# vani-nag/OWLRayTracing

Hardware: AMD Instinct MI355X
Metric: kNN queries/sec (10M pts, k=10) (higher is better)
Workload: dtype f32; 1 GPU; TrueKNN on 10000000 uniform-random 3-D points (numpy default_rng(0), [0,1)^3), k=10, start radius 0.25*(k/n)^(1/3)=0.0025; BASELINE.json configs[1]; ranks=1, n_points_total=10000000, k=10, kernel=team_kernel, parallelism=1 GPU

## Files before the change

### owlraytracing_amd/csrc/team_args.h

```cpp
#pragma once
#include <stdint.h>

#include <algorithm>
#include <cstdlib>

#include "lbvh.h"
#include "owlknn.h"

#ifndef TKNN_DIAG_BUILD
#define TKNN_DIAG_BUILD 0
#endif

namespace owlmi {

constexpr int kTeamBlock = 64;
inline int grab_for(int64_t count, int blocks, int turns, int cap) {
  if (const char *g = getenv("TKNN_GRAB")) return std::max(1, atoi(g));
  return (int)std::max<int64_t>(1, std::min<int64_t>(cap, count / ((int64_t)std::max(1, blocks) * 4 * turns)));
}
#ifndef TKNN_NREG3
#define TKNN_NREG3 1
#endif
inline int nreg_for(int k) { return k <= 16 ? 1 : (k <= 32 ? 2 : (k <= 48 && TKNN_NREG3 ? 3 : 4)); }

struct TeamArgs {
  LbvhView bvh, halo;
  LbvhWideView wide[2];
  float start_radius;
  const float *start_radii;
  int k;
  int max_rounds;
  int allow_unfinished;
  int first_step;
  int first_ext;
  int merge_ext;
  int count_flat_max;
  int lite;
  float tie_span;
  int diag;
  int32_t ngroups;
  int32_t *out_idx;
  float *out_dist;
  int64_t *out_isect;
  tknnNeigh *out_fb;
  int32_t *out_level;
  uint8_t *done;
  int64_t *isect_sorted;
  int32_t *next_level;
  uint8_t *tie;
  int32_t *tie_list;
  const uint8_t *skip;
  int32_t skip_is;
  const int32_t *slot_count;
  int grab;
  const int32_t *row_slot;
  unsigned long long *counters;
};

}
```

### owlraytracing_amd/csrc/trueknn_team.hip

```cpp
#include "knn_thresholds.h"
#include "team_args.h"
#include "team_lanes.h"
#include "team_walk.h"
#include "trueknn_engine.h"

#include <algorithm>
#include <cmath>
#include <cstdio>
#include <cstdlib>
#include <cstring>
#include <type_traits>

namespace owlmi {

namespace {

#ifndef TKNN_MAX_BLOCKS_3
#define TKNN_MAX_BLOCKS_3 256
#endif
#ifndef TKNN_MAX_BLOCKS_4
#define TKNN_MAX_BLOCKS_4 512
#endif
constexpr int max_blocks(int nreg) { return nreg == 4 ? TKNN_MAX_BLOCKS_4 : (nreg == 3 ? TKNN_MAX_BLOCKS_3 : 256); }
#ifndef TKNN_MAX_PER_QUERY
// ... 17 lines not shown
}
#ifndef TKNN_SORT_FIRST
#define TKNN_SORT_FIRST 1
#endif
#ifndef TKNN_TEAM_WAVES
#define TKNN_TEAM_WAVES 4
#endif
constexpr int kXcdCounter = kDbStats, kXcdCounterStride = 32;
constexpr int kTeamStack = 192;
constexpr int kQrecStride = 6;
constexpr int kScanBudget = 16384;
constexpr int kMaxStep = 2;
constexpr int kCountFlatGroups = 3;
constexpr int kLdsQrec = 64 * kQrecStride * 4;
constexpr int kLdsCnt = 64 * 2 * 4;
constexpr int kLdsList = 64 * 4 + 16;
constexpr int kLdsStack = kTeamStack * 4;
constexpr int kLdsShared = (kLdsCnt + kLdsList) > kLdsStack ? (kLdsCnt + kLdsList) : kLdsStack;
constexpr int kLdsSharedPadded = (kLdsShared + 15) & ~15;
constexpr int kCandCap = kCandCapacity;
template <int NREG>
struct TeamLayout {
  static constexpr int kMaxPerQuery = max_per_query(NREG);
  static constexpr int kMaxBlocks = max_blocks(NREG);
  static constexpr int kLdsBlk = kMaxBlocks * 4;
  static constexpr int kLdsMask = 64 * kMaxPerQuery;
  static constexpr int kHiWords = kMaxBlocks > 256 ? (kMaxPerQuery + 31) / 32 : 0;
  static constexpr int kLdsHi = 64 * kHiWords * 4;
  static constexpr int kEntStride = kMaxPerQuery + 4;
  static constexpr int kLdsEnt = 4 * kEntStride * 4;
  static constexpr int kLdsCand = 4 * kCandCap * 8;
  static constexpr int kOffMask = kLdsQrec + kLdsBlk;
  static constexpr int kOffHi = kOffMask + kLdsMask;
  static constexpr int kOffShared = kOffHi + kLdsHi;
  static constexpr int kOffEnt = kOffShared + kLdsSharedPadded;
  static constexpr int kOffCand = kOffEnt + kLdsEnt;
  static constexpr int kTeamLds = kOffCand + kLdsCand;
  static_assert(kEntStride % 4 == 0 && kOffEnt % 16 == 0, "entry lists must be 16-byte aligned");
  static_assert(kLdsMask % 4 == 0, "the ninth bits are words");
  static_assert(kMaxPerQuery <= 124 && kMaxPerQuery / 4 < 32, "list-length buckets of the pass lists are one bit each of a 32-bit word");
};

struct TeamLds {
  float *qrec;
  int32_t *blk;
  uint8_t *qblk;
  uint32_t *qhi;
  uint32_t *qcnt;
  int32_t *qlist;
  int32_t *ent;
  unsigned long long *cand;
};

template <bool SELECT, bool HALO, int NREG, bool FULL, bool TWO>
__device__ __forceinline__ void team_pass(const TeamArgs &a, const TeamLds &L, int n_list, int32_t first_slot,
                                          const LbvhPoint *own_pts, const LbvhPoint *halo_pts, int lane) {
  const int team = lane >> 4, tl = lane & 15;
  constexpr int kMaxPerQuery = TeamLayout<NREG>::kMaxPerQuery, kEntStride = TeamLayout<NREG>::kEntStride;
  static_assert(!(SELECT && TWO), "only a COUNT pass serves two levels");
  n_list = __builtin_amdgcn_readfirstlane(n_list);
  [[maybe_unused]] unsigned long long tp[4] = {0, 0, 0, 0};
  for (int r0 = 0; r0 < n_list; r0 += 4) {
    [[maybe_unused]] unsigned long long tp_mark = 0;
    if (TKNN_DIAG_BUILD && (a.diag & 128)) tp_mark = __builtin_amdgcn_s_memtime();
#define TP_LAP(i)                                                     \
  do {                                                                \
    if (TKNN_DIAG_BUILD && (a.diag & 128)) {                          \
      const unsigned long long now_ = __builtin_amdgcn_s_memtime();   \
      tp[i] += now_ - tp_mark;                                        \
      tp_mark = now_;                                                 \
    }                                                                 \
  } while (0)
    const bool on = r0 + team < n_list;
    int qi = 0;
    if (on) qi = L.qlist[r0 + team];
    bool lite_q = false;
    if (SELECT && NREG == 1) {
      lite_q = (qi >> 8) != 0;
      qi &= 0xff;
    }
    if (TKNN_DIAG_BUILD && SELECT && (a.diag & 128)) {
      const unsigned long long q_m = __ballot(on && tl == 0), l_m = __ballot(on && tl == 0 && lite_q);
      if (lane == 0) {
        atomicAdd(&a.counters[18], 1ull);
        atomicAdd(&a.counters[19], (unsigned long long)__popcll(q_m));
        atomicAdd(&a.counters[20], (unsigned long long)__popcll(l_m));
      }
    }
    const float *rec = L.qrec + qi * kQrecStride;
    const float t_qx = rec[0], t_qy = rec[1], t_qz = rec[2];
    const int32_t t_qid = __float_as_int(rec[3]);
    const float t_r = rec[4];
    const float t_mg = (fmaxf(fmaxf(fabsf(t_qx), fabsf(t_qy)), fabsf(t_qz)) + 2.0f * t_r) * 4.76837158203125e-07f;
    const float in_below = t_r - t_mg, in_upto = t_r + t_mg;
    const float r_inner = t_r * 0.5f;
    const float i0_below = r_inner - t_mg, i0_upto = r_inner + t_mg;
    uint32_t cnt_i0 = 0;
    const int packed = __float_as_int(rec[5]);
    [[maybe_unused]] int32_t out_row = 0;
    if (SELECT) out_row = a.bvh.prim_id[first_slot + qi];
    const int my_n = on ? (packed & 0xff) : 0;
    const int steps = max(max((int)__builtin_amdgcn_readlane(my_n, 0), (int)__builtin_amdgcn_readlane(my_n, 16)),
                          max((int)__builtin_amdgcn_readlane(my_n, 32), (int)__builtin_amdgcn_readlane(my_n, 48)));
    if (TKNN_DIAG_BUILD && (a.diag & 16) && lane == 0) atomicAdd(&a.counters[15], (unsigned long long)steps);
    const uint8_t *mine = L.qblk + qi * kMaxPerQuery;
    const int last = my_n - 1;
    const int32_t nan_block = a.wide[0].count[0];
    const int own_pos = (packed >> 8) & 0xff;
    const int n_near = (packed >> 16) & 0xff;
    const int last_near = n_near ? n_near - 1 : last;
    const int both = min(own_pos, last_near - own_pos);
    const bool right_longer = last_near - own_pos > own_pos;
    auto list_pos = [&](int it) -> int {
      if (!SELECT) return it;
      const int half = (it + 1) >> 1;
      const int alt = (it & 1) ? half : -half;
      const int far = it - both;
      const int off = it <= 2 * both ? alt : (right_longer ? far : -far);
      return it > last_near ? it : own_pos + off;
    };
    auto list_entry = [&](int pos) -> int32_t {
      int lp = list_pos(pos);
      if (n_near && lp >= n_near) lp = kMaxPerQuery - 1 - (lp - n_near);
      const int at = min(max(lp, 0), kMaxPerQuery - 1);
      int slot_at = mine[at];
      if (TeamLayout<NREG>::kHiWords) slot_at |= (int)((L.qhi[qi * TeamLayout<NREG>::kHiWords + (at >> 5)] >> (at & 31)) & 1u) << 8;
      int32_t e = L.blk[slot_at];
      if (TKNN_DIAG_BUILD && (a.diag & 64)) e = L.blk[mine[0]];
      return resolve_entry<HALO>(pos <= last ? e : nan_block);
    };
    const int steps4 = (steps + 3) & ~3;
    int32_t *my_ent = L.ent + team * kEntStride;
    const bool lite_round = SELECT && NREG == 1 && steps <= a.count_flat_max && __ballot(on && !lite_q) == 0ull;
    if (lite_round) {
      static_assert(4 * kCountFlatGroups + 4 <= 16, "one entry per lane of the team, the group of prefetch included");
      int32_t e = L.blk[mine[tl]];
      if (TKNN_DIAG_BUILD && (a.diag & 64)) e = L.blk[mine[0]];
      my_ent[tl] = resolve_entry<HALO>(tl <= last ? e : nan_block);
    } else {
      for (int base = 0; base < steps4 + 4; base += 16)
        if (base + tl < kEntStride) my_ent[base + tl] = list_entry(base + tl);
    }
    t_wave_sync();
    uint32_t cnt = 0;
    uint32_t bd[NREG], bi[NREG];
#pragma unroll
    for (int j = 0; j < NREG; j++) {
      bd[j] = 0x7f7fffffu;
      bi[j] = 0u;
    }
    constexpr bool full = FULL;
    uint32_t left_out = 0xffffffffu;
    auto kth_dist = [&]() -> float {
      uint32_t reg = bd[0];
#pragma unroll
      for (int j = 1; j < NREG; j++) reg = ((a.k - 1) >> 4) == j ? bd[j] : reg;
      return __uint_as_float(t_lane_read(reg, (team << 4) + ((a.k - 1) & 15)));
    };
    float tau2 = INFINITY;
    bool dirty = false;
    uint32_t fill_n = 0;
    auto merge_buffer = [&]() {
      t_wave_sync();
      t_merge_rows<NREG>(bd, bi, left_out, full, L.cand + team * kCandCap, fill_n, tl);
      t_wave_sync();
      fill_n = 0;
      dirty = false;
      tau2 = knn_gate_from_worst(kth_dist());
    };
    auto in_box = [&](const LbvhPoint &p, float t, float radius, float below, float upto) -> unsigned long long {
      unsigned long long in_m = __ballot(t <= below);
      const unsigned long long maybe = __ballot(t <= upto);
      if (__builtin_expect(maybe != in_m, 0)) in_m |= maybe & __ballot(knn_in_box(p.x, p.y, p.z, radius, t_qx, t_qy, t_qz));
      return in_m;
    };
    auto process = [&](const LbvhPoint &p, bool own_block = false) {
      const float dx = p.x - t_qx, dy = p.y - t_qy, dz = p.z - t_qz;
      const float t = fmaxf(fmaxf(fabsf(dx), fabsf(dy)), fabsf(dz));
      const unsigned long long in_m = in_box(p, t, t_r, in_below, in_upto);
      cnt = t_count_keep(cnt, in_m, p.id);
      if (TWO) cnt_i0 = t_count(cnt_i0, in_box(p, t, r_inner, i0_below, i0_upto));
      if (SELECT) {
        const float d2 = t_dist2(dx, dy, dz);
        unsigned long long pm = in_m & __ballot(d2 <= tau2);
        if (own_block) pm &= __ballot(p.id != t_qid);
        if (TKNN_DIAG_BUILD && (a.diag & 1)) pm = 0;
        if (pm) {
          if (TKNN_DIAG_BUILD && (a.diag & 16) && lane == 0) atomicAdd(&a.counters[26], (unsigned long long)__popcll(pm));
          const uint32_t mine16 = (uint32_t)(pm >> (team << 4)) & 0xffffu;
          if ((mine16 >> tl) & 1u) {
            const unsigned long long key = ((unsigned long long)__float_as_uint(d2) << 32) | (uint32_t)p.id;
            L.cand[team * kCandCap + fill_n + __popc(mine16 & ((1u << tl) - 1u))] = key;
          }
          fill_n += __popc(mine16);
          dirty = true;
          if (__ballot(fill_n >= 16u) != 0ull) {
            if (TKNN_DIAG_BUILD && (a.diag & 16) && lane == 0) atomicAdd(&a.counters[27], 1ull);
            merge_buffer();
          }
        }
      }
    };
    const LbvhPoint *own_base = a.bvh.points;
    const uint32_t lane_bytes = (uint32_t)tl * (uint32_t)sizeof(LbvhPoint);
    typedef int32_t t_int4 __attribute__((ext_vector_type(4)));
    const t_int4 *my_groups = (const t_int4 *)my_ent;
    auto fetch = [&](int32_t entry) -> t_point4 {
      const LbvhPoint p = load_block_point<HALO>(own_pts, halo_pts, entry, own_base, lane_bytes);
      return t_point4{p.x, p.y, p.z, __int_as_float(p.id)};
    };
// ... 105 lines not shown
        b2 = fetch(g.z);
        __builtin_amdgcn_sched_barrier(0);
        b3 = fetch(g.w);
        __builtin_amdgcn_sched_barrier(0);
      }
      for (int it = 0; it < steps; it += 4) {
        const t_int4 g = my_groups[(it >> 2) + 1];
        if (SELECT && it == 0) {
          if (NREG == 1 && TKNN_SORT_FIRST == 0)
            process(unpack(b0), true);
          else
            sort_first(unpack(b0));
        } else {
          process(unpack(b0));
        }
        b0 = fetch(g.x);
        process(unpack(b1));
        b1 = fetch(g.y);
        process(unpack(b2));
        b2 = fetch(g.z);
        process(unpack(b3));
        b3 = fetch(g.w);
        if (SELECT && dirty && __ballot(fill_n >= (uint32_t)TKNN_MERGE_AT) != 0ull) {
          if (TKNN_DIAG_BUILD && (a.diag & 16) && lane == 0) atomicAdd(&a.counters[27], 1ull);
          merge_buffer();
        }
        TP_LAP(it == 0 ? 1 : 2);
      }
    }
    if (SELECT && dirty) {
      if (TKNN_DIAG_BUILD && (a.diag & 16) && lane == 0) atomicAdd(&a.counters[27], 1ull);
      merge_buffer();
    }
    if (SELECT && full) {
      uint32_t v = left_out;
      v = min(v, (uint32_t)__builtin_amdgcn_update_dpp(-1, (int)v, 0x128 , 0xf, 0xf, false));
      v = min(v, (uint32_t)__builtin_amdgcn_update_dpp(-1, (int)v, 0x124 , 0xf, 0xf, false));
      v = min(v, (uint32_t)__builtin_amdgcn_update_dpp(-1, (int)v, 0x122 , 0xf, 0xf, false));
      v = min(v, (uint32_t)__builtin_amdgcn_update_dpp(-1, (int)v, 0x121 , 0xf, 0xf, false));
      left_out = v;
    }
    cnt = t_team_sum(cnt);
    const uint32_t self = cnt ? 1u : 0u;
    const uint32_t others = cnt - self;
    if (TWO) cnt_i0 = t_team_sum(cnt_i0);
    uint32_t tied = 0u;
    if (SELECT) {
      bool tie[NREG];
      bool any = false;
#pragma unroll
      for (int j = 0; j < NREG; j++) {
        uint32_t before = t_team_shr1(bd[j]);
        if (j > 0) before |= t_dpp<0x121>(bd[j - 1]) & (tl == 0 ? 0xffffffffu : 0u);
        tie[j] = ((j > 0) | (tl >= 1)) & (16 * j + tl <= a.k) & (bd[j] == before);
        if (full && j == NREG - 1) tie[j] |= (tl == 15) & (left_out == bd[j]);
        any |= tie[j];
      }
      if (__ballot(any) != 0ull) {
        const float qmax = fmaxf(fmaxf(fabsf(t_qx), fabsf(t_qy)), fabsf(t_qz));
        any = false;
        bool edge = false;
        const float q_r0 = a.start_radii ? a.start_radii[a.bvh.prim_id[first_slot + qi]] : a.start_radius;
#pragma unroll
        for (int j = 0; j < NREG; j++) {
          const bool t = tie[j] && tie_may_straddle(__uint_as_float(bd[j]), q_r0, t_r, qmax, a.tie_span);
          any |= t;
          edge |= t && (16 * j + tl == a.k || (full && j == NREG - 1 && tl == 15 && left_out == bd[j]));
        }
        if (on && edge) knn_note_tie_edge(a.tie, first_slot + qi);
      }
      tied = ((uint32_t)(__ballot(any) >> (team * 16)) & 0xffffu) ? 1u : 0u;
    }
    if (on && tl == 0) {
      uint32_t *out = L.qcnt + qi * 2;
      if (!TWO) {
        out[0] = cnt;
        out[1] = (self << 31) | (tied << 30);
      } else {
        out[0] = cnt_i0;
        out[1] = cnt | (self << 31);
      }
    }
    if (SELECT) {
      if (on && others >= (uint32_t)a.k) {
#pragma unroll
        for (int reg = 0; reg < NREG; reg++) {
          const int j = tl + 16 * reg;
          if (j >= a.k) continue;
          const int64_t o = (int64_t)out_row * a.k + j;
          const int32_t prim = knn_key_prim(((uint64_t)bd[reg] << 32) | bi[reg]);
          const float d = __uint_as_float(bd[reg]);
          if (a.out_idx) a.out_idx[o] = prim;
          if (a.out_dist) a.out_dist[o] = d;
          if (a.out_fb) {
            int2 *rec8 = (int2 *)(a.out_fb + o);
            rec8[0] = make_int2(prim, __float_as_int(d));
            rec8[1] = make_int2(j == 0 ? 0 : a.k, 0);
            if (j != 0) {
              int zero;
              asm volatile("v_mov_b32 %0, 0" : "=v"(zero));
              rec8[2] = make_int2(zero, zero);
            }
          }
        }
      }
    }
    TP_LAP(3);
  }
#undef TP_LAP
  if (TKNN_DIAG_BUILD && (a.diag & 128) && lane == 0)
    for (int i = 0; i < 4; i++) atomicAdd(&a.counters[(SELECT ? 36 : 28) + i], tp[i]);
}

template <bool HALO, int NREG, bool FULL>
__global__ void __launch_bounds__(kTeamBlock) __attribute__((amdgpu_waves_per_eu(TKNN_TEAM_WAVES))) team_kernel(TeamArgs a) {
  extern __shared__ __align__(16) unsigned char smem[];
  const int lane = threadIdx.x & 63;
  const int wid = threadIdx.x >> 6;
  const int tl = lane & 15;
  using Lay = TeamLayout<NREG>;
  constexpr int kMaxPerQuery = Lay::kMaxPerQuery;
  unsigned char *base = smem + wid * Lay::kTeamLds;
  float *qrec = (float *)base;
  int32_t *blk = (int32_t *)(base + kLdsQrec);
  uint8_t *qblk = (uint8_t *)(base + Lay::kOffMask);
  uint32_t *qhi = (uint32_t *)(base + Lay::kOffHi);
  constexpr int kMaxBlocks = Lay::kMaxBlocks;
  uint32_t *qcnt = (uint32_t *)(base + Lay::kOffShared);
  int32_t *qlist = (int32_t *)(base + Lay::kOffShared + kLdsCnt);
  int32_t *stack = (int32_t *)(base + Lay::kOffShared);
  int32_t *ent = (int32_t *)(base + Lay::kOffEnt);
  unsigned long long *cand = (unsigned long long *)(base + Lay::kOffCand);

  const LbvhPoint *own_pts = a.bvh.points + tl, *halo_pts = a.halo.points ? a.halo.points + tl : a.bvh.points + tl;
  unsigned long long my_isect_sum = 0, wave_node_tests = 0, wave_point_tests = 0;
  uint32_t my_levels = 0, my_unfinished = 0;
  int wave_levels = 0, wave_err = 0;
  uint32_t my_handed = 0;
  [[maybe_unused]] unsigned long long diag_scanned = 0, diag_listed = 0;
  int wave_min_handover = 0x7fffffff;
#if TKNN_DIAG_BUILD
  unsigned long long ph[5] = {0, 0, 0, 0, 0}, t_mark = __builtin_amdgcn_s_memtime();
#define PHASE_END(i)                                         \
  do {                                                       \
    const unsigned long long now_ = __builtin_amdgcn_s_memtime(); \
    ph[i] += now_ - t_mark;                                  \
    t_mark = now_;                                           \
  } while (0)
#else
#define PHASE_END(i) \
  do {               \
  } while (0)
#endif

  const int xcc = (int)__builtin_amdgcn_s_getreg(6164 ) & 7;
  const int chunk = max(1, min(1024, a.ngroups / 128));
  uint32_t seg_empty = 0;
  for (;;) {
    int g = -1;
    for (int t = 0; t < 8 && g < 0; t++) {
      const int x = (xcc + t) & 7;
      if (seg_empty & (1u << x)) continue;
      int v = 0;
      if (lane == 0) v = (int)atomicAdd(&a.counters[kXcdCounter + kXcdCounterStride * x], 1ull);
      v = __builtin_amdgcn_readfirstlane(v);
      const int cand = ((v / chunk) * 8 + x) * chunk + (v % chunk);
      if (cand < a.ngroups)
        g = cand;
// ... 112 lines not shown
      };
      float *node_boxes = (float *)ent;
      static_assert(64 * 6 * 4 <= Lay::kLdsEnt + Lay::kLdsCand, "the gather's child boxes borrow the entry lists' LDS");
      auto stash_boxes = [&](const LbvhBox &bx) {
        float2 *dst = (float2 *)(node_boxes + 6 * lane);
        dst[0] = make_float2(bx.lo[0], bx.lo[1]);
        dst[1] = make_float2(bx.lo[2], bx.hi[0]);
        dst[2] = make_float2(bx.hi[1], bx.hi[2]);
        t_wave_sync();
      };
      struct ChildBox {
        float2 w0, w1, w2;
      };
      auto child_box = [&](int src) -> ChildBox {
        int boff;
        asm("s_mul_i32 %0, %1, 24" : "=s"(boff) : "s"(src));
        const float2 *b = (const float2 *)((const char *)node_boxes + boff);
        return ChildBox{b[0], b[1], b[2]};
      };
      auto gap_to_me = [&](const ChildBox &c) -> float {
        return separation(c.w0.x, c.w0.y, c.w1.x, c.w1.y, c.w2.x, c.w2.y, q.x, q.y, q.z, q.x, q.y, q.z);
      };
      auto for_children_ahead = [&](unsigned long long mask, bool top_down, auto test) {
        auto take = [&](int last) -> int {
          if (!mask) return last;
          const int src = top_down ? 63 - __builtin_clzll(mask) : __ffsll((long long)mask) - 1;
          mask &= ~(1ull << src);
          return src;
        };
        if (!mask) return;
        int s0 = take(0), s1;
        ChildBox c0 = child_box(s0), c1;
        for (;;) {
          bool more = mask != 0ull;
          s1 = take(s0);
          c1 = child_box(s1);
          if (!test(s0, c0) || !more) break;
          more = mask != 0ull;
          s0 = take(s1);
          c0 = child_box(s0);
          if (!test(s1, c1) || !more) break;
        }
      };

      PHASE_END(0);
      my_own_pos = 0;
      int cur = 0;
      uint8_t *my_list = qblk + lane * kMaxPerQuery;
      if (Lay::kHiWords) {
#pragma unroll
        for (int w = 0; w < Lay::kHiWords; w++) qhi[lane * Lay::kHiWords + w] = 0u;
      }
      int nb = 0, scanned = 0;
      for (int tree = 0; tree < 2 && !too_big; tree++) {
        const LbvhWideView &wv = a.wide[tree];
        const int32_t tree_n = tree == 0 ? a.bvh.n : a.halo.n;
        if (tree_n <= 0 || wv.levels <= 0) continue;
        int sp = 0, nleaf = 0;
        if (lane == 0) stack[wv.levels > 1 ? 0 : kTeamStack - 1] = (wv.levels << 26) | 0;
        if (wv.levels > 1)
          sp = 1;
        else
          nleaf = 1;
        t_wave_sync();
        const int32_t last_block = wv.count[0] - 1;
        while ((sp > 0 || nleaf > 0) && !too_big) {
          if (sp > 0 && sp + nleaf + 63 <= kTeamStack) {
            const int32_t e = __builtin_amdgcn_readfirstlane(stack[sp - 1]);
            sp--;
            const int lvl = (e >> 26) - 1;
            const int32_t first_child = (e & 0x3ffffff) * 64;
            const int32_t c = first_child + lane;
            const bool valid = lvl == wv.levels - 1 ? (lane < wv.count[lvl] && first_child == 0) : (c < wv.count[lvl]);
            LbvhBox bx = {{0.f, 0.f, 0.f}, {0.f, 0.f, 0.f}};
            if (valid) bx = wv.level[lvl][c];
            wave_node_tests += 64;
            const bool ov = valid & overlaps_packet(bx);
            const unsigned long long om = __ballot(ov);
            const int cnt = __popcll(om);
            if (lvl > 1) {
              if (ov) stack[sp + t_rank(om)] = (lvl << 26) | c;
              sp += cnt;
            } else {
              if (om) stash_boxes(bx);
              for_children_ahead(om, true, [&](int src, const ChildBox &box) -> bool {
                if (__ballot(gap_to_me(box) <= reach_walk) == 0ull) return true;
                if (lane == 0) stack[kTeamStack - 1 - nleaf] = (lvl << 26) | (first_child + src);
                nleaf++;
                return true;
              });
            }
            t_wave_sync();
            continue;
          }
          if (nleaf == 0) {
            too_big = true;
            break;
          }
          auto leaf_boxes = [&](int i) -> LbvhBox {
            const int32_t e = __builtin_amdgcn_readfirstlane(stack[kTeamStack - nleaf + (i < nleaf ? i : nleaf - 1)]);
            return wv.level[0][min((e & 0x3ffffff) * 64 + lane, last_block)];
          };
          LbvhBox bx_next = leaf_boxes(0);
          for (int i = 0; i < nleaf && !too_big; i++) {
            const int32_t e = __builtin_amdgcn_readfirstlane(stack[kTeamStack - nleaf + i]);
            const int32_t first_child = (e & 0x3ffffff) * 64;
            const LbvhBox bx = bx_next;
// ... 8 lines not shown
              too_big = true;
              break;
            }
            if (om) stash_boxes(bx);
            for_children_ahead(om, false, [&](int src, const ChildBox &box) -> bool {
              const float gap = gap_to_me(box);
              bool need = gap <= reach_walk;
              if (TKNN_DIAG_BUILD && (a.diag & 8)) need = false;
              if (__ballot(need) == 0ull) return true;
              if (nb >= kMaxBlocks) {
                too_big = true;
                return false;
              }
              const int32_t block = first_child + src;
              blk[nb] = (int32_t)((uint32_t)block | ((uint32_t)tree << 31));
              if (tree == 0 && (uint32_t)(block - g * 4) < 4u && block == (slot >> 4)) my_own_pos = cur & 0xffff;
              if (need) {
                const bool inner = gap <= reach_step;
                const int at = inner ? (cur & 0xffff) : kMaxPerQuery - 1 - (cur >> 16);
                const int at_c = min(max(at, 0), kMaxPerQuery - 1);
                my_list[at_c] = (uint8_t)nb;
                if (Lay::kHiWords && nb >= 256) qhi[lane * Lay::kHiWords + (at_c >> 5)] |= 1u << (at_c & 31);
                cur += inner ? 1 : 0x10000;
              }
              nb++;
              return true;
            });
          }
          nleaf = 0;
          t_wave_sync();
        }
        t_wave_sync();
      }
      if (TKNN_DIAG_BUILD && (a.diag & 32)) diag_listed += nb;
      n_in = cur & 0xffff, n_out = cur >> 16;
      if (ext) {
        if (too_big || __ballot(n_in + n_out > kMaxPerQuery) != 0ull) {
          ext = false;
          ext_ok = false;
          too_big = false;
          t_wave_sync();
          continue;
        }
        reuse = __ballot(active) != 0ull;
      }
      my_nblk = n_in;
      if (!ext) n_out = 0;
      break;
      }
      if (NREG < 3) {
        if (__ballot(my_nblk > kMaxPerQuery) != 0ull) too_big = true;
        if (too_big) {
          if (active) {
            a.done[slot] = 0;
            a.isect_sorted[slot] = isect;
            a.next_level[slot] = level;
            my_handed++;
          }
          wave_min_handover = min(wave_min_handover, level);
          active = false;
          break;
        }
      } else if (too_big || __ballot(my_nblk > kMaxPerQuery) != 0ull) {
        const bool hand_over = active && (too_big || my_nblk > kMaxPerQuery);
        if (hand_over) {
          a.done[slot] = 0;
          a.isect_sorted[slot] = isect;
          a.next_level[slot] = level;
          my_handed++;
          active = false;
        }
        wave_min_handover = min(wave_min_handover, level);
        if (__ballot(active) == 0ull) break;
      }
      const int my_packed = my_nblk | (my_own_pos << 8) | (my_nblk > n_in ? n_in << 16 : n_out << 24);
      qrec[lane * kQrecStride + 5] = __int_as_float(my_packed);

      PHASE_END(1);
      const bool speculate = m == 1 && active && !served && level > 0 && prev_others * 8u >= (uint32_t)(a.k + a.k / 2);
      const bool count_first = active && !served && !speculate;
      served = false;
      constexpr int kLiteBuckets = NREG == 1 ? kCountFlatGroups + 1 : 0;
      static_assert(kMaxPerQuery / 4 + kLiteBuckets < 32, "list-length buckets of the pass lists are one bit each of a 32-bit word");
      auto build_qlist = [&](bool sel, int nblk, bool lite) -> int {
        const int bucket = lite ? nblk >> 2 : (nblk >> 2) + kLiteBuckets;
        if (lane == 0) qlist[64] = 0;
        t_wave_sync();
        if (sel) __hip_atomic_fetch_or((uint32_t *)&qlist[64], 1u << bucket, __ATOMIC_RELAXED, __HIP_MEMORY_SCOPE_WAVEFRONT);
        t_wave_sync();
        uint32_t present = (uint32_t)__builtin_amdgcn_readfirstlane(qlist[64]);
        int base = 0, pos = 0;
        while (present) {
          const int b = __ffs((int)present) - 1;
          present &= present - 1u;
          const bool mine = sel && bucket == b;
          const unsigned long long bm = __ballot(mine);
          if (mine) pos = base + t_rank(bm);
          base += __popcll(bm);
        }
        if (sel) qlist[pos] = lite ? lane | 0x100 : lane;
        t_wave_sync();
        return base;
      };
      {
        const int n_count = build_qlist(count_first, my_nblk, false);
        if (!(TKNN_DIAG_BUILD && (a.diag & 4))) {
          if (m > 1)
            team_pass<false, HALO, NREG, false, true>(a, L, n_count, g * 64, own_pts, halo_pts, lane);
          else
            team_pass<false, HALO, NREG, false, false>(a, L, n_count, g * 64, own_pts, halo_pts, lane);
        }
        t_wave_sync();
      }
      PHASE_END(2);
      uint32_t c0 = 0, c1 = 0, selfc = 0;
      int fin_at = -1;
      if (count_first) {
        c0 = qcnt[lane * 2 + 0];
        const uint32_t w1 = qcnt[lane * 2 + 1];
        c1 = m > 1 ? (w1 & 0x3fffffffu) : 0u;
        selfc = w1 >> 31;
        if (c0 - selfc >= (uint32_t)a.k)
          fin_at = 0;
        else if (m > 1 && c1 - selfc >= (uint32_t)a.k)
          fin_at = 1;
      }
      int sel_nblk = my_nblk;
      if (reuse && a.merge_ext && count_first && fin_at < 0 && ((m > 1 ? c1 : c0) - selfc) * 8u >= (uint32_t)(a.k + a.k / 2)) {
        fin_at = m;
        const int pk = __float_as_int(qrec[lane * kQrecStride + 5]);
        sel_nblk = (pk & 0xff) + ((pk >> 24) & 0xff);
        qrec[lane * kQrecStride + 4] = qrec[lane * kQrecStride + 4] * 2.0f;
        qrec[lane * kQrecStride + 5] = __int_as_float(sel_nblk | (pk & 0xff00) | ((pk & 0xff) << 16) | (pk & (int)0xff000000u));
      }
      const bool select_now = speculate || fin_at >= 0;
      if (m > 1 && fin_at == 0) qrec[lane * kQrecStride + 4] = r_in0;
      bool lite = false;
      if (NREG == 1 && a.lite && fin_at >= 0 && fin_at < m) {
        const int pk = __float_as_int(qrec[lane * kQrecStride + 5]);
        lite = (fin_at == 0 ? c0 : c1) - selfc <= 16u && (pk & 0xff0000) == 0 && (pk & 0xff) <= a.count_flat_max;
      }
      {
        t_wave_sync();
        const int n_select = build_qlist(select_now, sel_nblk, lite);
        if (!(TKNN_DIAG_BUILD && (a.diag & 2))) team_pass<true, HALO, NREG, FULL, false>(a, L, n_select, g * 64, own_pts, halo_pts, lane);
        t_wave_sync();
      }
      PHASE_END(3);
      if (TKNN_DIAG_BUILD && lite && qcnt[lane * 2 + 0] != (fin_at == 0 ? c0 : c1)) atomicAdd(&a.counters[21], 1ull);
      const bool ext_sel = fin_at == m;
      bool finished = fin_at >= 0 && !ext_sel;
      uint32_t last_others = prev_others;
      if (speculate) {
        c0 = qcnt[lane * 2 + 0];
        selfc = qcnt[lane * 2 + 1] >> 31;
        finished = c0 - selfc >= (uint32_t)a.k;
        fin_at = finished ? 0 : -1;
      }
      uint32_t c_ext = 0, n_back = 0;
      if (ext_sel) {
        c_ext = qcnt[lane * 2 + 0];
        finished = c_ext - selfc >= (uint32_t)a.k;
        const int pk = __float_as_int(qrec[lane * kQrecStride + 5]);
        n_back = ((uint32_t)pk >> 24) & 0xffu;
        qrec[lane * kQrecStride + 5] = __int_as_float(pk & 0x00ffffff);
      }
      int levels_run = 0;
      if (count_first || speculate) {
        levels_run = finished || ext_sel ? fin_at + 1 : m;
        isect += c0;
        if (levels_run > 1) isect += c1;
        isect += c_ext;
        my_levels += (uint32_t)levels_run;
        last_others = ext_sel ? c_ext - selfc : (m > 1 ? c1 : c0) - selfc;
        prev_others = last_others;
      }
      wave_levels = max(wave_levels, (int)t_wave_max((float)(active ? level + levels_run : 0)));
      {
        const unsigned long long passes = (count_first ? 1ull : 0ull) + (select_now ? 1ull : 0ull);
        wave_point_tests += t_wave_sum(((unsigned long long)my_nblk * passes + n_back) * LBVH_BLOCK);
      }
      if (finished) {
        my_isect_sum += (unsigned long long)isect;
        if (a.out_isect) a.out_isect[row] = isect;
        if (a.out_fb) a.out_fb[(int64_t)row * a.k].intersections = isect;
        const int fin_level = level + (fin_at > 0 ? fin_at : 0);
        if (a.out_level) a.out_level[row] = fin_level;
        if ((qcnt[lane * 2 + 1] >> 30) & 1u) knn_flag_tie(a.tie, a.tie_list, a.counters, slot, fin_level, 2);
      }
      active = active && !finished;
      int m_done = m;
      if (reuse && a.merge_ext) {
        if (__ballot(active && !ext_sel) == 0ull) {
          m_done = m + 1;
          reuse = false;
        } else {
          served = ext_sel;
        }
      }
      level += m_done;
      t_wave_sync();
      if (__ballot(active) == 0ull) break;
      if (level >= a.max_rounds) {
        if (!a.allow_unfinished) wave_err |= 1;
        break;
      }
      for (int j = 0; j < m_done; j++) r = r * 2.0f;
      {
        const float pmax = t_wave_max(active ? (float)last_others : 0.f);
        float expect = pmax * 8.f;
        step = 1;
        while (step < kMaxStep && expect < 0.5f * (float)a.k) {
          step++;
          expect *= 8.f;
        }
        ext_next = ext_ok && expect < 2.5f * (float)a.k ? 1 : 0;
      }
    }
    if (active) my_unfinished++;
  }

  const unsigned long long isum = t_wave_sum(my_isect_sum), lsum = t_wave_sum((unsigned long long)my_levels), usum = t_wave_sum((unsigned long long)my_unfinished),
                           hsum = t_wave_sum((unsigned long long)my_handed);
  if (lane == 0) {
    unsigned long long *st = a.counters + kStatBase + (blockIdx.x & (kStatStripes - 1)) * kStatStride;
    atomicMax(&st[1], (unsigned long long)wave_levels);
    atomicAdd(&st[2], wave_node_tests);
    atomicAdd(&st[3], wave_point_tests);
    atomicAdd(&st[4], isum);
    atomicAdd(&st[6], lsum);
    if (usum) atomicAdd(&st[7], usum);
    if (hsum) {
      atomicAdd(&st[8], hsum);
      atomicMin(&st[9], (unsigned long long)wave_min_handover);
    }
    if (wave_err) atomicOr(&st[5], (unsigned long long)wave_err);
#if TKNN_DIAG_BUILD
    for (int i = 0; i < 5; i++) atomicAdd(&a.counters[10 + i], ph[i]);
    if (a.diag & 32) {
      atomicAdd(&a.counters[24], diag_scanned);
      atomicAdd(&a.counters[25], diag_listed);
    }
#endif
  }
}


__global__ void __launch_bounds__(256) team_prep_kernel(uint8_t *done, uint8_t *tie, int64_t n, unsigned long long *counters, int32_t *levels) {
  const int64_t tid = (int64_t)blockIdx.x * blockDim.x + threadIdx.x, nth = (int64_t)gridDim.x * blockDim.x;
  if (tid < kCounters + 8 * kXcdCounterStride) counters[tid] = tid == 9 ? ~0ull : 0ull;
  if (tid < kStatStripes * kStatStride) counters[kStatBase + tid] = (tid & (kStatStride - 1)) == 9 ? ~0ull : 0ull;
  const int64_t words = n / 16;
  uint4 *d16 = reinterpret_cast<uint4 *>(done), *t16 = reinterpret_cast<uint4 *>(tie);
  const uint4 ones = make_uint4(0x01010101u, 0x01010101u, 0x01010101u, 0x01010101u), zeros = make_uint4(0u, 0u, 0u, 0u);
  for (int64_t i = tid; i < words; i += nth) {
    d16[i] = ones;
    t16[i] = zeros;
  }
  for (int64_t i = words * 16 + tid; i < n; i += nth) {
    done[i] = 1;
    tie[i] = 0;
  }
  if (levels)
    for (int64_t i = tid; i < n; i += nth) levels[i] = -1;
}

}

bool Engine::team_kernel_supports(int k) { return k >= 1 && k <= 64; }


int Engine::first_step_estimate(const SolveArgs &sa) const {
  float radius = sa.start_radius;
  for (int m = 1; m < 3; m++) {
    if (expected_box_population(radius) >= 0.5 * sa.k) return m;
    radius *= 2.0f;
  }
  return 3;
}

bool Engine::solve_team(const SolveArgs &sa, tknnSolveInfo *info, hipStream_t s) {
  const int64_t n = bvh_.size();
  if (n >= (1ll << 28)) return false;
  TeamArgs a = team_args(sa);
  set_solve_args(a, sa);
  a.first_step = sa.d_start_radii ? 1 : first_step_estimate(sa);
  {
    float radius = sa.start_radius;
    for (int t = 1; t < std::min(a.first_step, kMaxStep); t++) radius *= 2.0f;
    a.first_ext = !sa.d_start_radii && expected_box_population(radius) < 2.5 * sa.k ? 1 : 0;
    if (const char *e = getenv("TKNN_TEAM_EXT")) a.first_ext = atoi(e) > 0 ? a.first_ext : -1;
    a.merge_ext = 1;
    if (const char *e = getenv("TKNN_TEAM_MERGE")) a.merge_ext = atoi(e) > 0 ? 1 : 0;
    a.count_flat_max = 4 * kCountFlatGroups;
    if (const char *e = getenv("TKNN_TEAM_COUNT_FLAT")) a.count_flat_max = std::max(0, std::min(atoi(e), 4 * kCountFlatGroups));
    a.lite = 1;
    if (const char *e = getenv("TKNN_TEAM_LITE")) a.lite = atoi(e) > 0 ? 1 : 0;
  }
  {
    int dims = 0;
    for (int ax = 0; ax < 3; ax++) dims += scene_[3 + ax] > scene_[ax] ? 1 : 0;
    if (halo_count() > 0) dims = 3;
    a.tie_span = dims >= 3 ? 1.73206f : (dims == 2 ? 1.41422f : 1.00001f);
  }
  if (TKNN_DIAG_BUILD)
    if (const char *d = getenv("TKNN_TEAM_DIAG")) a.diag = atoi(d);
  a.ngroups = (int32_t)((n + 63) / 64);

  const int nreg = nreg_for(sa.k);
  const char *walk_all = getenv("TKNN_TEAM_WALK_ALL");
  if (sa.k > 32 && walk_all && atoi(walk_all)) {
    reset_solve_state(sa.d_levels, s);
    const tknnSolveInfo all = walk(sa, a, 4, nullptr, (int32_t)n, 0, false, s);
    if (info) *info = all;
    return true;
  }
  int per_cu = 2;
  static_assert(kDbStripes * kDbStripeWords >= 8 * kXcdCounterStride, "the packet counters borrow the words of RT-DBSCAN's striped statistics");
  const size_t lds = (size_t)kTeamBlock / 64 * (size_t)(nreg == 1 ? TeamLayout<1>::kTeamLds : (nreg == 2 ? TeamLayout<2>::kTeamLds
                                                         : (nreg == 3 ? TeamLayout<3>::kTeamLds : TeamLayout<4>::kTeamLds)));
  const bool full_list = sa.k == 16 * nreg;
  using TeamEntry = void (*)(TeamArgs);
  static const TeamEntry entries[2][4][2] = {
      {{team_kernel<false, 1, false>, team_kernel<false, 1, true>}, {team_kernel<false, 2, false>, team_kernel<false, 2, true>},
       {team_kernel<false, 3, false>, team_kernel<false, 3, true>}, {team_kernel<false, 4, false>, team_kernel<false, 4, true>}},
      {{team_kernel<true, 1, false>, team_kernel<true, 1, true>}, {team_kernel<true, 2, false>, team_kernel<true, 2, true>},
       {team_kernel<true, 3, false>, team_kernel<true, 3, true>}, {team_kernel<true, 4, false>, team_kernel<true, 4, true>}}};
  const TeamEntry entry = entries[halo_count() > 0 ? 1 : 0][nreg - 1][full_list ? 1 : 0];
  if (hipOccupancyMaxActiveBlocksPerMultiprocessor(&per_cu, (const void *)entry, kTeamBlock, lds) != hipSuccess) per_cu = 2;
  per_cu = std::max(1, std::min(per_cu, lds_workgroups_per_cu(lds)));
  if (const char *cap = getenv("TKNN_TEAM_WAVES_PER_CU"))
    per_cu = std::max(1, std::min(per_cu, atoi(cap)));
  const int64_t want = (a.ngroups + kTeamBlock / 64 - 1) / (kTeamBlock / 64);
  const int blocks = (int)std::max<int64_t>(1, std::min<int64_t>(want, (int64_t)cu_count_ * per_cu));

  hipLaunchKernelGGL(team_prep_kernel, dim3(cu_count_ * 4), dim3(256), 0, s, done_, tie_, n, counters_, sa.phase >= 2 ? nullptr : sa.d_levels);
  OWLMI_HIP(hipEventRecord(ev_a_, s));
  {
    void *kargs[] = {(void *)&a};
    OWLMI_HIP(hipLaunchKernel((const void *)entry, dim3(blocks), dim3(kTeamBlock), kargs, lds, s));
  }
  OWLMI_HIP(hipGetLastError());
  OWLMI_HIP(hipEventRecord(ev_b_, s));
  launch_tie_fix(sa, tie_list_, -1, std::min(cu_count_ * 4, kTieListCap / 4), s);
  OWLMI_HIP(hipEventRecord(ev_c_, s));
  fetch_stat_stripes(s);
  OWLMI_HIP(hipMemcpyAsync(h_counters_ + 10, counters_ + kTieCounter, 3 * sizeof(unsigned long long), hipMemcpyDeviceToHost, s));
  OWLMI_HIP(hipStreamSynchronize(s));
  const KernelStats st = fold_stat_stripes(true);
  float ms = 0;
  OWLMI_HIP(hipEventElapsedTime(&ms, ev_a_, ev_b_));
  if (st.handed_over == 0 && h_counters_[10] <= (unsigned long long)kTieListCap) {
    ties_early_ = true;
    early_tie_rows_ = (int64_t)h_counters_[10];
    early_tie_left_ = (int64_t)h_counters_[12];
    OWLMI_HIP(hipEventElapsedTime(&early_tie_ms_, ev_b_, ev_c_));
  }
#if TKNN_DIAG_BUILD
  if (getenv("TKNN_TEAM_DIAG")) {
    unsigned long long t[5];
    OWLMI_HIP(hipMemcpy(t, counters_ + 10, sizeof t, hipMemcpyDeviceToHost));
    const double tot = (double)(t[0] + t[1] + t[2] + t[3] + t[4]);
    unsigned long long wave_steps = 0;
    OWLMI_HIP(hipMemcpy(&wave_steps, counters_ + 15, sizeof wave_steps, hipMemcpyDeviceToHost));
    fprintf(stderr, "[team diag] block steps: %.3g wave steps x 4 teams for %.3g listed blocks (lockstep efficiency %.1f%%)\n",
            (double)wave_steps, (double)st.point_tests / LBVH_BLOCK, 100.0 * ((double)st.point_tests / LBVH_BLOCK) / (4.0 * (double)wave_steps));
    if (a.diag & 16) {
      unsigned long long g[2];
      OWLMI_HIP(hipMemcpy(g, counters_ + 26, sizeof g, hipMemcpyDeviceToHost));
      fprintf(stderr, "[team diag] inserts: %.4g candidates passed the gate after the sorted first block (%.2f per query), in %.4g lock-step rounds of the wave (%.2f per query)\n",
              (double)g[0], (double)g[0] / (double)n, (double)g[1], (double)g[1] / (double)n);
    }
    if (a.diag & 128) {
      unsigned long long g[12];
      OWLMI_HIP(hipMemcpy(g, counters_ + 28, sizeof g, hipMemcpyDeviceToHost));
      for (int pass = 0; pass < 2; pass++) {
        const unsigned long long *t4 = g + 8 * pass;
        const double tt = (double)(t4[0] + t4[1] + t4[2] + t4[3]);
        fprintf(stderr, "[team diag] %s pass, wave time: %.3g cycles in all; set-up %.1f%%  first group %.1f%%  other groups %.1f%%  epilogue %.1f%%\n",
                pass ? "SELECT" : "COUNT", tt, 100 * t4[0] / tt, 100 * t4[1] / tt, 100 * t4[2] / tt, 100 * t4[3] / tt);
      }
      unsigned long long lt[6];
      OWLMI_HIP(hipMemcpy(lt, counters_ + 16, sizeof lt, hipMemcpyDeviceToHost));
      fprintf(stderr, "[team diag] SELECT rounds: %.4g with %.4g queries, %.4g of them light; light rounds: %.4g (%.1f%% of the rounds) with %.4g queries; "
                      "light queries whose SELECT count differs from COUNT's: %llu\n",
              (double)lt[2], (double)lt[3], (double)lt[4], (double)lt[0], lt[2] ? 100.0 * (double)lt[0] / (double)lt[2] : 0.0, (double)lt[1], lt[5]);
    }
    if (a.diag & 32) {
      unsigned long long g[2];
      OWLMI_HIP(hipMemcpy(g, counters_ + 24, sizeof g, hipMemcpyDeviceToHost));
      fprintf(stderr, "[team diag] gather: %.3g leaf blocks tested against the 64 queries, %.3g of them listed (%.1f%%)\n", (double)g[0], (double)g[1], 100.0 * (double)g[1] / (double)g[0]);
    }
    fprintf(stderr, "[team diag] mean busy time per wave %.2f ms of %.2f ms kernel time (%d waves; s_memtime at 100 MHz)\n",
// ... 36 lines not shown
```

Measured before the change: 2.143 billion queries/s.

## Add specialized plain team kernel with constexpr args and scalar-held pointers

Adds a PlainTeamArgs variant of the team kernel's argument struct for the common case: a single own tree, k <= 16, no halo, default knobs. Unused fields and toggles become compile-time constants, so the branches and loads that depend on them fold away. Output pointers, k and the start radius are pinned to scalar registers via readfirstlane, and slot/row values are kept in vector registers, with the aim of cutting register and scalar-load pressure. This adds an extra kernel instantiation and dispatch logic, and silently drops to the generic path whenever any knob environment variable is set.

```diff
diff --git a/owlraytracing_amd/csrc/team_args.h b/owlraytracing_amd/csrc/team_args.h
--- a/owlraytracing_amd/csrc/team_args.h
+++ b/owlraytracing_amd/csrc/team_args.h
@@ -3,6 +3,7 @@
 
 #include <algorithm>
 #include <cstdlib>
+#include <type_traits>
 
 #include "lbvh.h"
 #include "owlknn.h"
@@ -57,4 +58,77 @@
   unsigned long long *counters;
 };
 
+struct PlainTeamArgs {
+  struct {
+    const LbvhPoint *points;
+    const int32_t *prim_id;
+    int32_t n;
+  } bvh;
+  struct NoTree {
+    static constexpr const LbvhPoint *points = nullptr;
+    static constexpr int32_t n = 0;
+  };
+  static constexpr NoTree halo = {};
+  LbvhWideView wide[1];
+  float start_radius;
+  static constexpr const float *start_radii = nullptr;
+  int k;
+  int max_rounds;
+  int allow_unfinished;
+  int first_step;
+  int first_ext;
+  static constexpr int merge_ext = 1;
+  static constexpr int count_flat_max = 12;
+  static constexpr int lite = 1;
+  float tie_span;
+  static constexpr int diag = 0;
+  int32_t ngroups;
+  int32_t *out_idx;
+  float *out_dist;
+  int64_t *out_isect;
+  static constexpr tknnNeigh *out_fb = nullptr;
+  static constexpr int32_t *out_level = nullptr;
+  uint8_t *done;
+  int64_t *isect_sorted;
+  int32_t *next_level;
+  uint8_t *tie;
+  int32_t *tie_list;
+  static constexpr const uint8_t *skip = nullptr;
+  static constexpr int32_t skip_is = 0;
+  unsigned long long *counters;
+};
+
+inline bool plain_team_solve(const TeamArgs &a) {
+  return a.out_idx && a.out_dist && a.out_isect && !a.out_fb && !a.out_level && !a.start_radii && !a.skip && a.halo.n <= 0 && !a.halo.points &&
+         a.merge_ext == PlainTeamArgs::merge_ext && a.lite == PlainTeamArgs::lite && a.count_flat_max == PlainTeamArgs::count_flat_max &&
+         a.diag == PlainTeamArgs::diag;
 }
+inline PlainTeamArgs plain_team_args(const TeamArgs &a) {
+  PlainTeamArgs p;
+  p.bvh.points = a.bvh.points;
+  p.bvh.prim_id = a.bvh.prim_id;
+  p.bvh.n = a.bvh.n;
+  p.wide[0] = a.wide[0];
+  p.start_radius = a.start_radius;
+  p.k = a.k;
+  p.max_rounds = a.max_rounds;
+  p.allow_unfinished = a.allow_unfinished;
+  p.first_step = a.first_step;
+  p.first_ext = a.first_ext;
+  p.tie_span = a.tie_span;
+  p.ngroups = a.ngroups;
+  p.out_idx = a.out_idx;
+  p.out_dist = a.out_dist;
+  p.out_isect = a.out_isect;
+  p.done = a.done;
+  p.isect_sorted = a.isect_sorted;
+  p.next_level = a.next_level;
+  p.tie = a.tie;
+  p.tie_list = a.tie_list;
+  p.counters = a.counters;
+  return p;
+}
+template <bool PLAIN>
+using TeamArgsOf = std::conditional_t<PLAIN, PlainTeamArgs, TeamArgs>;
+
+}
diff --git a/owlraytracing_amd/csrc/trueknn_team.hip b/owlraytracing_amd/csrc/trueknn_team.hip
--- a/owlraytracing_amd/csrc/trueknn_team.hip
+++ b/owlraytracing_amd/csrc/trueknn_team.hip
@@ -93,12 +93,51 @@
   unsigned long long *cand;
 };
 
-template <bool SELECT, bool HALO, int NREG, bool FULL, bool TWO>
-__device__ __forceinline__ void team_pass(const TeamArgs &a, const TeamLds &L, int n_list, int32_t first_slot,
+__device__ __forceinline__ uint32_t t_hold_word(uint32_t w) {
+  asm volatile("" : "+v"(w));
+  return (uint32_t)__builtin_amdgcn_readfirstlane((int)w);
+}
+template <class T>
+__device__ __forceinline__ void t_hold(T &v) {
+  static_assert(sizeof(T) == 4 || sizeof(T) == 8, "a word or a pointer");
+  uint32_t w[sizeof(T) / 4];
+  memcpy(w, &v, sizeof(T));
+  for (size_t i = 0; i < sizeof(T) / 4; i++) w[i] = t_hold_word(w[i]);
+  memcpy(&v, w, sizeof(T));
+}
+
+__device__ __forceinline__ int t_lane_again(int lane) {
+  asm volatile("" : "+v"(lane));
+  return lane;
+}
+
+template <bool PLAIN>
+struct TeamHeld {};
+template <>
+struct TeamHeld<true> {
+  int32_t *out_idx;
+  float *out_dist;
+  int64_t *out_isect;
+  uint8_t *tie;
+  float start_radius;
+  int k;
+};
+
+template <bool PLAIN>
+__device__ __forceinline__ int team_k(const TeamArgsOf<PLAIN> &a, const TeamHeld<PLAIN> &held) {
+  if constexpr (PLAIN)
+    return held.k;
+  else
+    return a.k;
+}
+
+template <bool SELECT, bool HALO, int NREG, bool FULL, bool TWO, bool PLAIN = false>
+__device__ __forceinline__ void team_pass(const TeamArgsOf<PLAIN> &a, const TeamHeld<PLAIN> &held, const TeamLds &L, int n_list, int32_t first_slot,
                                           const LbvhPoint *own_pts, const LbvhPoint *halo_pts, int lane) {
   const int team = lane >> 4, tl = lane & 15;
   constexpr int kMaxPerQuery = TeamLayout<NREG>::kMaxPerQuery, kEntStride = TeamLayout<NREG>::kEntStride;
   static_assert(!(SELECT && TWO), "only a COUNT pass serves two levels");
+#define TEAM_K team_k<PLAIN>(a, held)
   n_list = __builtin_amdgcn_readfirstlane(n_list);
   [[maybe_unused]] unsigned long long tp[4] = {0, 0, 0, 0};
   for (int r0 = 0; r0 < n_list; r0 += 4) {
@@ -195,8 +234,8 @@
     auto kth_dist = [&]() -> float {
       uint32_t reg = bd[0];
 #pragma unroll
-      for (int j = 1; j < NREG; j++) reg = ((a.k - 1) >> 4) == j ? bd[j] : reg;
-      return __uint_as_float(t_lane_read(reg, (team << 4) + ((a.k - 1) & 15)));
+      for (int j = 1; j < NREG; j++) reg = ((TEAM_K - 1) >> 4) == j ? bd[j] : reg;
+      return __uint_as_float(t_lane_read(reg, (team << 4) + ((TEAM_K - 1) & 15)));
     };
     float tau2 = INFINITY;
     bool dirty = false;
@@ -408,7 +447,7 @@
       for (int j = 0; j < NREG; j++) {
         uint32_t before = t_team_shr1(bd[j]);
         if (j > 0) before |= t_dpp<0x121>(bd[j - 1]) & (tl == 0 ? 0xffffffffu : 0u);
-        tie[j] = ((j > 0) | (tl >= 1)) & (16 * j + tl <= a.k) & (bd[j] == before);
+        tie[j] = ((j > 0) | (tl >= 1)) & (16 * j + tl <= TEAM_K) & (bd[j] == before);
         if (full && j == NREG - 1) tie[j] |= (tl == 15) & (left_out == bd[j]);
         any |= tie[j];
       }
@@ -416,14 +455,23 @@
         const float qmax = fmaxf(fmaxf(fabsf(t_qx), fabsf(t_qy)), fabsf(t_qz));
         any = false;
         bool edge = false;
-        const float q_r0 = a.start_radii ? a.start_radii[a.bvh.prim_id[first_slot + qi]] : a.start_radius;
+        float q_r0;
+        if constexpr (PLAIN)
+          q_r0 = held.start_radius;
+        else
+          q_r0 = a.start_radii ? a.start_radii[a.bvh.prim_id[first_slot + qi]] : a.start_radius;
 #pragma unroll
         for (int j = 0; j < NREG; j++) {
           const bool t = tie[j] && tie_may_straddle(__uint_as_float(bd[j]), q_r0, t_r, qmax, a.tie_span);
           any |= t;
-          edge |= t && (16 * j + tl == a.k || (full && j == NREG - 1 && tl == 15 && left_out == bd[j]));
-        }
-        if (on && edge) knn_note_tie_edge(a.tie, first_slot + qi);
+          edge |= t && (16 * j + tl == TEAM_K || (full && j == NREG - 1 && tl == 15 && left_out == bd[j]));
+        }
+        if (on && edge) {
+          if constexpr (PLAIN)
+            knn_note_tie_edge(held.tie, first_slot + qi);
+          else
+            knn_note_tie_edge(a.tie, first_slot + qi);
+        }
       }
       tied = ((uint32_t)(__ballot(any) >> (team * 16)) & 0xffffu) ? 1u : 0u;
     }
@@ -438,20 +486,25 @@
       }
     }
     if (SELECT) {
-      if (on && others >= (uint32_t)a.k) {
+      if (on && others >= (uint32_t)TEAM_K) {
 #pragma unroll
         for (int reg = 0; reg < NREG; reg++) {
           const int j = tl + 16 * reg;
-          if (j >= a.k) continue;
-          const int64_t o = (int64_t)out_row * a.k + j;
+          if (j >= TEAM_K) continue;
+          const int64_t o = (int64_t)out_row * TEAM_K + j;
           const int32_t prim = knn_key_prim(((uint64_t)bd[reg] << 32) | bi[reg]);
           const float d = __uint_as_float(bd[reg]);
-          if (a.out_idx) a.out_idx[o] = prim;
-          if (a.out_dist) a.out_dist[o] = d;
+          if constexpr (PLAIN) {
+            held.out_idx[o] = prim;
+            held.out_dist[o] = d;
+          } else {
+            if (a.out_idx) a.out_idx[o] = prim;
+            if (a.out_dist) a.out_dist[o] = d;
+          }
           if (a.out_fb) {
             int2 *rec8 = (int2 *)(a.out_fb + o);
             rec8[0] = make_int2(prim, __float_as_int(d));
-            rec8[1] = make_int2(j == 0 ? 0 : a.k, 0);
+            rec8[1] = make_int2(j == 0 ? 0 : TEAM_K, 0);
             if (j != 0) {
               int zero;
               asm volatile("v_mov_b32 %0, 0" : "=v"(zero));
@@ -468,8 +521,21 @@
     for (int i = 0; i < 4; i++) atomicAdd(&a.counters[(SELECT ? 36 : 28) + i], tp[i]);
 }
 
-template <bool HALO, int NREG, bool FULL>
-__global__ void __launch_bounds__(kTeamBlock) __attribute__((amdgpu_waves_per_eu(TKNN_TEAM_WAVES))) team_kernel(TeamArgs a) {
+template <bool HALO, int NREG, bool FULL, bool PLAIN = false>
+__global__ void __launch_bounds__(kTeamBlock) __attribute__((amdgpu_waves_per_eu(TKNN_TEAM_WAVES))) team_kernel(TeamArgsOf<PLAIN> a) {
+  static_assert(!PLAIN || (!HALO && NREG == 1), "the plain kernel: one own tree, k <= 16");
+  static_assert(PlainTeamArgs::count_flat_max == 4 * kCountFlatGroups, "a plain solve's flat COUNT rounds are the generic solve's");
+  TeamHeld<PLAIN> held;
+  if constexpr (PLAIN) {
+    held.out_idx = a.out_idx, held.out_dist = a.out_dist, held.out_isect = a.out_isect, held.tie = a.tie;
+    held.start_radius = a.start_radius, held.k = a.k;
+    t_hold(held.out_idx);
+    t_hold(held.out_dist);
+    t_hold(held.out_isect);
+    t_hold(held.tie);
+    t_hold(held.start_radius);
+    t_hold(held.k);
+  }
   extern __shared__ __align__(16) unsigned char smem[];
   const int lane = threadIdx.x & 63;
   const int wid = threadIdx.x >> 6;
@@ -688,7 +754,7 @@
         for (int w = 0; w < Lay::kHiWords; w++) qhi[lane * Lay::kHiWords + w] = 0u;
       }
       int nb = 0, scanned = 0;
-      for (int tree = 0; tree < 2 && !too_big; tree++) {
+      for (int tree = 0; tree < (PLAIN ? 1 : 2) && !too_big; tree++) {
         const LbvhWideView &wv = a.wide[tree];
         const int32_t tree_n = tree == 0 ? a.bvh.n : a.halo.n;
         if (tree_n <= 0 || wv.levels <= 0) continue;
@@ -803,9 +869,11 @@
         if (__ballot(my_nblk > kMaxPerQuery) != 0ull) too_big = true;
         if (too_big) {
           if (active) {
-            a.done[slot] = 0;
-            a.isect_sorted[slot] = isect;
-            a.next_level[slot] = level;
+            int32_t slot_now = slot;
+            if constexpr (PLAIN) slot_now = g * 64 + t_lane_again(lane);
+            a.done[slot_now] = 0;
+            a.isect_sorted[slot_now] = isect;
+            a.next_level[slot_now] = level;
             my_handed++;
           }
           wave_min_handover = min(wave_min_handover, level);
@@ -828,7 +896,7 @@
       qrec[lane * kQrecStride + 5] = __int_as_float(my_packed);
 
       PHASE_END(1);
-      const bool speculate = m == 1 && active && !served && level > 0 && prev_others * 8u >= (uint32_t)(a.k + a.k / 2);
+      const bool speculate = m == 1 && active && !served && level > 0 && prev_others * 8u >= (uint32_t)(TEAM_K + TEAM_K / 2);
       const bool count_first = active && !served && !speculate;
       served = false;
       constexpr int kLiteBuckets = NREG == 1 ? kCountFlatGroups + 1 : 0;
@@ -857,9 +925,9 @@
         const int n_count = build_qlist(count_first, my_nblk, false);
         if (!(TKNN_DIAG_BUILD && (a.diag & 4))) {
           if (m > 1)
-            team_pass<false, HALO, NREG, false, true>(a, L, n_count, g * 64, own_pts, halo_pts, lane);
+            team_pass<false, HALO, NREG, false, true, PLAIN>(a, held, L, n_count, g * 64, own_pts, halo_pts, lane);
           else
-            team_pass<false, HALO, NREG, false, false>(a, L, n_count, g * 64, own_pts, halo_pts, lane);
+            team_pass<false, HALO, NREG, false, false, PLAIN>(a, held, L, n_count, g * 64, own_pts, halo_pts, lane);
         }
         t_wave_sync();
       }
@@ -871,13 +939,13 @@
         const uint32_t w1 = qcnt[lane * 2 + 1];
         c1 = m > 1 ? (w1 & 0x3fffffffu) : 0u;
         selfc = w1 >> 31;
-        if (c0 - selfc >= (uint32_t)a.k)
+        if (c0 - selfc >= (uint32_t)TEAM_K)
           fin_at = 0;
-        else if (m > 1 && c1 - selfc >= (uint32_t)a.k)
+        else if (m > 1 && c1 - selfc >= (uint32_t)TEAM_K)
           fin_at = 1;
       }
       int sel_nblk = my_nblk;
-      if (reuse && a.merge_ext && count_first && fin_at < 0 && ((m > 1 ? c1 : c0) - selfc) * 8u >= (uint32_t)(a.k + a.k / 2)) {
+      if (reuse && a.merge_ext && count_first && fin_at < 0 && ((m > 1 ? c1 : c0) - selfc) * 8u >= (uint32_t)(TEAM_K + TEAM_K / 2)) {
         fin_at = m;
         const int pk = __float_as_int(qrec[lane * kQrecStride + 5]);
         sel_nblk = (pk & 0xff) + ((pk >> 24) & 0xff);
@@ -894,7 +962,7 @@
       {
         t_wave_sync();
         const int n_select = build_qlist(select_now, sel_nblk, lite);
-        if (!(TKNN_DIAG_BUILD && (a.diag & 2))) team_pass<true, HALO, NREG, FULL, false>(a, L, n_select, g * 64, own_pts, halo_pts, lane);
+        if (!(TKNN_DIAG_BUILD && (a.diag & 2))) team_pass<true, HALO, NREG, FULL, false, PLAIN>(a, held, L, n_select, g * 64, own_pts, halo_pts, lane);
         t_wave_sync();
       }
       PHASE_END(3);
@@ -905,13 +973,13 @@
       if (speculate) {
         c0 = qcnt[lane * 2 + 0];
         selfc = qcnt[lane * 2 + 1] >> 31;
-        finished = c0 - selfc >= (uint32_t)a.k;
+        finished = c0 - selfc >= (uint32_t)TEAM_K;
         fin_at = finished ? 0 : -1;
       }
       uint32_t c_ext = 0, n_back = 0;
       if (ext_sel) {
         c_ext = qcnt[lane * 2 + 0];
-        finished = c_ext - selfc >= (uint32_t)a.k;
+        finished = c_ext - selfc >= (uint32_t)TEAM_K;
         const int pk = __float_as_int(qrec[lane * kQrecStride + 5]);
         n_back = ((uint32_t)pk >> 24) & 0xffu;
         qrec[lane * kQrecStride + 5] = __int_as_float(pk & 0x00ffffff);
@@ -933,11 +1001,24 @@
       }
       if (finished) {
         my_isect_sum += (unsigned long long)isect;
-        if (a.out_isect) a.out_isect[row] = isect;
-        if (a.out_fb) a.out_fb[(int64_t)row * a.k].intersections = isect;
+        if constexpr (PLAIN) {
+          int32_t row_now = row;
+          asm volatile("" : "+v"(row_now));
+          held.out_isect[row_now] = isect;
+        } else if (a.out_isect) {
+          a.out_isect[row] = isect;
+        }
+        if (a.out_fb) a.out_fb[(int64_t)row * TEAM_K].intersections = isect;
         const int fin_level = level + (fin_at > 0 ? fin_at : 0);
         if (a.out_level) a.out_level[row] = fin_level;
-        if ((qcnt[lane * 2 + 1] >> 30) & 1u) knn_flag_tie(a.tie, a.tie_list, a.counters, slot, fin_level, 2);
+        if ((qcnt[lane * 2 + 1] >> 30) & 1u) {
+          if constexpr (PLAIN) {
+            const int32_t slot_now = g * 64 + t_lane_again(lane);
+            knn_flag_tie(held.tie, a.tie_list, a.counters, slot_now, fin_level, 2);
+          } else {
+            knn_flag_tie(a.tie, a.tie_list, a.counters, slot, fin_level, 2);
+          }
+        }
       }
       active = active && !finished;
       int m_done = m;
@@ -961,11 +1042,11 @@
         const float pmax = t_wave_max(active ? (float)last_others : 0.f);
         float expect = pmax * 8.f;
         step = 1;
-        while (step < kMaxStep && expect < 0.5f * (float)a.k) {
+        while (step < kMaxStep && expect < 0.5f * (float)TEAM_K) {
           step++;
           expect *= 8.f;
         }
-        ext_next = ext_ok && expect < 2.5f * (float)a.k ? 1 : 0;
+        ext_next = ext_ok && expect < 2.5f * (float)TEAM_K ? 1 : 0;
       }
     }
     if (active) my_unfinished++;
@@ -996,6 +1077,8 @@
   }
 }
 
+
+#undef TEAM_K
 
 __global__ void __launch_bounds__(256) team_prep_kernel(uint8_t *done, uint8_t *tie, int64_t n, unsigned long long *counters, int32_t *levels) {
   const int64_t tid = (int64_t)blockIdx.x * blockDim.x + threadIdx.x, nth = (int64_t)gridDim.x * blockDim.x;
@@ -1077,8 +1160,16 @@
        {team_kernel<false, 3, false>, team_kernel<false, 3, true>}, {team_kernel<false, 4, false>, team_kernel<false, 4, true>}},
       {{team_kernel<true, 1, false>, team_kernel<true, 1, true>}, {team_kernel<true, 2, false>, team_kernel<true, 2, true>},
        {team_kernel<true, 3, false>, team_kernel<true, 3, true>}, {team_kernel<true, 4, false>, team_kernel<true, 4, true>}}};
-  const TeamEntry entry = entries[halo_count() > 0 ? 1 : 0][nreg - 1][full_list ? 1 : 0];
-  if (hipOccupancyMaxActiveBlocksPerMultiprocessor(&per_cu, (const void *)entry, kTeamBlock, lds) != hipSuccess) per_cu = 2;
+  using PlainEntry = void (*)(PlainTeamArgs);
+  static const PlainEntry plain_entries[2] = {team_kernel<false, 1, false, true>, team_kernel<false, 1, true, true>};
+  bool plain = nreg == 1 && halo_count() == 0 && plain_team_solve(a);
+  for (const char *knob : {"TKNN_TEAM_MERGE", "TKNN_TEAM_LITE", "TKNN_TEAM_COUNT_FLAT", "TKNN_TEAM_EXT", "TKNN_TEAM_DIAG"})
+    if (getenv(knob)) plain = false;
+  if (const char *e = getenv("TKNN_TEAM_PLAIN")) plain = plain && atoi(e) > 0;
+  const PlainTeamArgs plain_a = plain_team_args(a);
+  if (getenv("TKNN_VERBOSE")) fprintf(stderr, "[team] packet kernel: the %s instantiation\n", plain ? "plain" : "generic");
+  const void *entry = plain ? (const void *)plain_entries[full_list ? 1 : 0] : (const void *)entries[halo_count() > 0 ? 1 : 0][nreg - 1][full_list ? 1 : 0];
+  if (hipOccupancyMaxActiveBlocksPerMultiprocessor(&per_cu, entry, kTeamBlock, lds) != hipSuccess) per_cu = 2;
   per_cu = std::max(1, std::min(per_cu, lds_workgroups_per_cu(lds)));
   if (const char *cap = getenv("TKNN_TEAM_WAVES_PER_CU"))
     per_cu = std::max(1, std::min(per_cu, atoi(cap)));
@@ -1088,8 +1179,8 @@
   hipLaunchKernelGGL(team_prep_kernel, dim3(cu_count_ * 4), dim3(256), 0, s, done_, tie_, n, counters_, sa.phase >= 2 ? nullptr : sa.d_levels);
   OWLMI_HIP(hipEventRecord(ev_a_, s));
   {
-    void *kargs[] = {(void *)&a};
-    OWLMI_HIP(hipLaunchKernel((const void *)entry, dim3(blocks), dim3(kTeamBlock), kargs, lds, s));
+    void *kargs[] = {plain ? (void *)&plain_a : (void *)&a};
+    OWLMI_HIP(hipLaunchKernel(entry, dim3(blocks), dim3(kTeamBlock), kargs, lds, s));
   }
   OWLMI_HIP(hipGetLastError());
   OWLMI_HIP(hipEventRecord(ev_b_, s));
```

Result: faster. 2.181 billion queries/s (median of 6 runs) (+1.8%).
